# nzfeng/signed-heat-3d

Measured on AMD Instinct MI355X. Metric: grid-nodes/sec end-to-end SHM (conv+PCG), higher is better.
Workload: dtype f64 (Step 1: f64 / packed-f32 tiers)

## Files before the change

### signed-heat-3d_amd/csrc/shm_conv_tiered.hip.h

```cpp
#pragma once
#include "shm_far_carry.h"
#include "shm_kernels.hip.h"

namespace shm {

typedef unsigned uint2v __attribute__((ext_vector_type(2)));
constexpr double kNearA1 = 3.384507729693224e-04;
__device__ __forceinline__ double yukawa_near(double x, double c1, double c2, double m1, const uint2v* __restrict__ tab) {
    const double y0 = __builtin_amdgcn_rsq(x);
    const double t = x * y0;
    const double e2 = fma(-t, y0, 1.0);
    const double cc = fma(e2, c2, c1);
    const double tm = fma(-t, cc, m1);
    const double kf = tm - m1;
    const unsigned ki = (unsigned)__double_as_longlong(tm);
    const double f = fma(-t, cc, -kf);
    const double q = y0 * cc;
    double p = 5.727446245172041e-08;
    p = fma(p, f, kNearA1);
    p = fma(p, f, 1.0);
    uint2v tv = tab[ki & 2047u];
    tv.y += ki << 9;
    return __builtin_bit_cast(double, tv) * (p * q);
}

template <int B>
__device__ __forceinline__ void yukawa_near_batch(const double* __restrict__ x, double c1, double c2, double m1, const uint2v* __restrict__ tab, double* __restrict__ g) {
    double y0[B], t[B], cc[B], q[B], tm[B], f[B], p[B];
    unsigned ki[B];
    uint2v tv[B];
#pragma unroll
    for (int b = 0; b < B; b++) y0[b] = __builtin_amdgcn_rsq(x[b]);
#pragma unroll
    for (int b = 0; b < B; b++) t[b] = x[b] * y0[b];
#pragma unroll
    for (int b = 0; b < B; b++) cc[b] = fma(fma(-t[b], y0[b], 1.0), c2, c1);
#pragma unroll
    for (int b = 0; b < B; b++) tm[b] = fma(-t[b], cc[b], m1);
#pragma unroll
    for (int b = 0; b < B; b++) {
        ki[b] = (unsigned)__double_as_longlong(tm[b]);
        tv[b] = tab[ki[b] & 2047u];
    }
#pragma unroll
    for (int b = 0; b < B; b++) q[b] = y0[b] * cc[b];
#pragma unroll
    for (int b = 0; b < B; b++) f[b] = fma(-t[b], cc[b], -(tm[b] - m1));
#pragma unroll
    for (int b = 0; b < B; b++) p[b] = fma(fma(5.727446245172041e-08, f[b], kNearA1), f[b], 1.0);
#pragma unroll
    for (int b = 0; b < B; b++) p[b] *= q[b];
#pragma unroll
    for (int b = 0; b < B; b++) {
        tv[b].y += ki[b] << 9;
        g[b] = __builtin_bit_cast(double, tv[b]) * p[b];
    }
}

#ifndef SHM_TIER_ASM_BCAST
#define SHM_TIER_ASM_BCAST 1
#endif
__device__ __forceinline__ void pk_fma_lo(float2v& acc, float2v w, float2v g) {
#if SHM_TIER_ASM_BCAST
    asm("v_pk_fma_f32 %0, %1, %2, %0 op_sel_hi:[0,1,1]" : "+v"(acc) : "v"(w), "v"(g));
#else
    acc = __builtin_elementwise_fma(float2v{w.x, w.x}, g, acc);
#endif
}
__device__ __forceinline__ void pk_fma_hi(float2v& acc, float2v w, float2v g) {
#if SHM_TIER_ASM_BCAST
    asm("v_pk_fma_f32 %0, %1, %2, %0 op_sel:[1,0,0] op_sel_hi:[1,1,1]" : "+v"(acc) : "v"(w), "v"(g));
#else
    acc = __builtin_elementwise_fma(float2v{w.y, w.y}, g, acc);
#endif
}

__device__ __forceinline__ int mask_rank(unsigned long long m) {
    return (int)__builtin_amdgcn_mbcnt_hi((unsigned)(m >> 32), __builtin_amdgcn_mbcnt_lo((unsigned)m, 0u));
}

__device__ __forceinline__ double exp2_tab(double u, const uint2v* __restrict__ tab) {
    const double tm = u + 6755399441055744.0;
    const unsigned ki = (unsigned)__double_as_longlong(tm);
    const double f = u - (tm - 6755399441055744.0);
    uint2v tv = tab[ki & 2047u];
    tv.y += ki << 9;
    return __builtin_bit_cast(double, tv) * fma(fma(5.727446245172041e-08, f, kNearA1), f, 1.0);
}

__device__ __forceinline__ float uniform_f32(float v) { return __int_as_float(__builtin_amdgcn_readfirstlane(__float_as_int(v))); }

__device__ __forceinline__ int sample_verdict(unsigned long long* ctr) {
    int v = 0;
    for (unsigned spins = 0; spins < (1u << 20); spins++) {
        v = __builtin_amdgcn_readfirstlane((int)__hip_atomic_load(ctr + 3, __ATOMIC_RELAXED, __HIP_MEMORY_SCOPE_AGENT));
        if (v != 0) break;
        __builtin_amdgcn_s_sleep(32);
    }
    if (v == 0) {
        int r = 0;
        if ((threadIdx.x & 63u) == 0u) {
            unsigned long long expected = 0ull;
            const bool won = __hip_atomic_compare_exchange_strong(ctr + 3, &expected, 2ull, __ATOMIC_RELAXED, __ATOMIC_RELAXED, __HIP_MEMORY_SCOPE_AGENT);
            r = won ? 2 : (int)expected;
        }
        v = __builtin_amdgcn_readfirstlane(r);
    }
    return v == 1;
}
__device__ __forceinline__ void sample_report(unsigned long long* ctr, unsigned long long far_pairs, unsigned long long redo_pairs, int sample_blocks) {
    __hip_atomic_fetch_add(ctr + 0, far_pairs, __ATOMIC_RELAXED, __HIP_MEMORY_SCOPE_AGENT);
    __hip_atomic_fetch_add(ctr + 1, redo_pairs, __ATOMIC_RELAXED, __HIP_MEMORY_SCOPE_AGENT);
    const unsigned long long before = __hip_atomic_fetch_add(ctr + 2, 1ull, __ATOMIC_RELEASE, __HIP_MEMORY_SCOPE_AGENT);
    if (before + 1ull == (unsigned long long)sample_blocks) {
        __builtin_amdgcn_fence(__ATOMIC_ACQUIRE, "agent");
        const unsigned long long farp = __hip_atomic_load(ctr + 0, __ATOMIC_RELAXED, __HIP_MEMORY_SCOPE_AGENT);
        const unsigned long long redo = __hip_atomic_load(ctr + 1, __ATOMIC_RELAXED, __HIP_MEMORY_SCOPE_AGENT);
        unsigned long long expected = 0ull;
        __hip_atomic_compare_exchange_strong(ctr + 3, &expected, (farp > 0ull && redo * 25ull <= farp) ? 1ull : 2ull, __ATOMIC_RELAXED, __ATOMIC_RELAXED, __HIP_MEMORY_SCOPE_AGENT);
    }
}

#ifndef SHM_TIER_TX
#define SHM_TIER_TX 8
#endif
constexpr int kTierTX = SHM_TIER_TX, kTierTY = 64 / kTierTX;
constexpr double kTierBudget = 1.0e-8, kTierEpsFar = 1.0e-6;
constexpr double kTierU0 = 24.0;
constexpr int kTierFlush = 256;
constexpr int kTierCluster = 64;
constexpr int kTierChunk = 4;
constexpr int kTierFill = kTierCluster * kTierChunk;

#ifndef SHM_TIER_FAR_UNROLL
#define SHM_TIER_FAR_UNROLL 4
#endif
#ifndef SHM_TIER_LDS_FETCH
#define SHM_TIER_LDS_FETCH 1
#endif
#ifndef SHM_TIER_LOOKAHEAD
#define SHM_TIER_LOOKAHEAD 1
#endif
#ifndef SHM_TIER_NEAR_BATCH
#define SHM_TIER_NEAR_BATCH 4
#endif
#ifndef SHM_TIER_WAVES_PER_EU
#define SHM_TIER_WAVES_PER_EU 2
#endif
template <int NPT, typename TY, bool CHECK>
__global__ __launch_bounds__(kBlock) __attribute__((amdgpu_waves_per_eu(SHM_TIER_WAVES_PER_EU, SHM_TIER_WAVES_PER_EU))) void conv_tiered_kernel(
    ConvParams P, const double* __restrict__ src , const float* __restrict__ clusters,
    const double* __restrict__ exp_tab_g , TY* __restrict__ Y0, TY* __restrict__ Y1, TY* __restrict__ Y2,
    unsigned long long* __restrict__ counters, unsigned* __restrict__ next_unit ) {
    static_assert(NPT % 2 == 0, "the far tier handles a lane's nodes in packed pairs");
    constexpr int kWaves = kBlock / kWave;
    constexpr int kFarUnroll = SHM_TIER_FAR_UNROLL;
    static_assert(kFarUnroll == kFarGroup, "the carry's bookkeeping (shm_far_carry.h) counts in groups of the far loop's unroll");
    constexpr int kFarList = kTierCluster + kFarGroup;
    static_assert((kTierCluster + kFarGroup - 1 + kFarGroup - 1) / kFarGroup * kFarGroup <= kFarList, "carry + cluster + padding fit the far lists");
    __shared__ double stage64[kWaves][kTierCluster * 6];
    __shared__ __attribute__((aligned(16))) float farA[kWaves][kFarList * 4];
    __shared__ __attribute__((aligned(16))) float farB[kWaves][kFarList * NPT];
    __shared__ __attribute__((aligned(16))) float farC[kWaves][kFarList * 2];
#if SHM_TIER_LDS_FETCH
    __shared__ double2 raw[kWaves][3][kTierCluster];
#endif
    __shared__ uint2v exp_tab[2048];
    __shared__ float4 star_stash[kWaves];
    const int wave = __builtin_amdgcn_readfirstlane((int)(threadIdx.x >> 6)), lane = (int)(threadIdx.x & 63);
    double* const tile = stage64[wave];
    float* const tA = farA[wave];
    float* const tB = farB[wave];
    float* const tC = farC[wave];
    for (int a = threadIdx.x; a < 2048; a += kBlock) {
        uint2v tv = __builtin_bit_cast(uint2v, exp_tab_g[a]);
        tv.y -= (unsigned)a << 9;
        exp_tab[a] = tv;
    }
    __syncthreads();
    const int n = P.n;
    const size_t plane = (size_t)n * n;
    const float lam_l2 = (float)(P.lambda * 1.4426950408889634);
    const float g_l2 = P.tier_log * 1.4426950408889634f;
    const bool drop_on = P.drop_eps_soft > 0.f;
    const float cellq = (float)(P.cell * (P.lambda * 1.4426950408889634));
    const float lws = uniform_f32((float)log2(P.wscale));
    constexpr double kHalfZ = 0.5 * (NPT - 1);
    constexpr double kHalfX = 0.5 * (kTierTX - 1), kHalfY = 0.5 * (kTierTY - 1);
    const float rt_w = (float)(sqrt(kHalfX * kHalfX + kHalfY * kHalfY + kHalfZ * kHalfZ) * P.cell) * 1.000001f;
    const float hx = uniform_f32((float)(kHalfX * P.cell) * 1.000001f), hy = uniform_f32((float)(kHalfY * P.cell) * 1.000001f),
                hz = uniform_f32((float)(kHalfZ * P.cell) * 1.000001f);
    const double c1 = -P.cexp, c2 = -0.5 * P.cexp;
    unsigned long long cnt_near = 0, cnt_far = 0, cnt_redo = 0;
    int decided = -1;
    const unsigned n_units = (unsigned)P.n_tiles;
    const unsigned per_q = (n_units + 7u) / 8u;
    const unsigned my_q = blockIdx.x & 7u;
    unsigned q_off = 0;
    for (;;) {
        unsigned unit = 0xffffffffu;
        while (q_off < 8u) {
            const unsigned q = (my_q + q_off) & 7u;
            const unsigned lo = q * per_q, hi = min(n_units, lo + per_q);
            unsigned t = 0;
            if (lane == 0) t = atomicAdd(next_unit + q, 1u);
            t = (unsigned)__builtin_amdgcn_readfirstlane((int)t);
            if (lo + t < hi) {
                unit = lo + t;
                break;
            }
            q_off++;
        }
        if (unit == 0xffffffffu) break;
        const int tzq = (int)(unit / (unsigned)(P.tiles_x * P.tiles_y)), trem = (int)unit - tzq * (P.tiles_x * P.tiles_y);
        const int tz = P.layer_order ? P.layer_order[tzq] : tzq;
        bool use_diff = false;
        int rule_sel = -1;
        if constexpr (CHECK) {
            use_diff = P.far_rule != 0;
            if (P.unit_rule) {
                rule_sel = (int)P.unit_rule[tzq];
                if (rule_sel == 2) {
                    if (decided < 0) decided = sample_verdict(P.sample_ctr);
                    use_diff = decided != 0;
                } else {
                    use_diff = rule_sel == 1;
                }
            }
        }
        const unsigned long long far_before = cnt_far, redo_before = cnt_redo;
        const int ty = trem / P.tiles_x, tx = trem - ty * P.tiles_x;
        const int i0 = tx * kTierTX, j0 = ty * kTierTY, kk0 = P.kk_begin + tz * NPT;

        double pz0 = 0., ax[NPT], ay[NPT], az[NPT];
        float qz0 = 0.f;
        float2v fx[NPT / 2], fy[NPT / 2], fz[NPT / 2];
        const int li = i0 + (lane % kTierTX), lj = j0 + (lane / kTierTX);
        const int ci = min(li, n - 1), cj = min(lj, n - 1);
        const double px = ci * P.cell + P.bbox_min[0], py = cj * P.cell + P.bbox_min[1];
        const float qx = (float)(px * (P.lambda * 1.4426950408889634)), qy = (float)(py * (P.lambda * 1.4426950408889634));
#pragma unroll
        for (int e = 0; e < NPT; e++) {
            ax[e] = ay[e] = az[e] = 0.;
            fx[e / 2] = fy[e / 2] = fz[e / 2] = float2v{0.f, 0.f};
        }
        pz0 = (P.k0 + kk0 - 1) * P.cell + P.bbox_min[2];
        {
            const long long b = __double_as_longlong(pz0);
            const unsigned lo = (unsigned)__builtin_amdgcn_readfirstlane((int)(unsigned)b), hi = (unsigned)__builtin_amdgcn_readfirstlane((int)(unsigned)(b >> 32));
            pz0 = __longlong_as_double((long long)(((unsigned long long)hi << 32) | lo));
        }
        qz0 = uniform_f32((float)(pz0 * (P.lambda * 1.4426950408889634)));
        const bool live_xy = li < n && lj < n;
        const float cx = uniform_f32((float)((i0 + kHalfX) * P.cell + P.bbox_min[0])), cy = uniform_f32((float)((j0 + kHalfY) * P.cell + P.bbox_min[1]));
        const float cz = uniform_f32((float)((P.k0 + kk0 - 1 + kHalfZ) * P.cell + P.bbox_min[2]));
        float dmin = 3.0e38f, wnear = 0.f, nx = 0.f, ny = 0.f, nz = 0.f;
        for (int s = lane; s < P.S; s += kWave) {
            const double* q = src + (size_t)s * 6;
            const float dx = cx - (float)q[0], dy = cy - (float)q[1], dz = cz - (float)q[2];
            const float w0 = (float)(q[3] * P.wscale), w1 = (float)(q[4] * P.wscale), w2c = (float)(q[5] * P.wscale);
            const float d2 = dx * dx + dy * dy + dz * dz, w2 = w0 * w0 + w1 * w1 + w2c * w2c;
            if (d2 < dmin || (d2 == dmin && w2 > wnear)) {
                dmin = d2;
                wnear = w2;
                nx = dx;
                ny = dy;
                nz = dz;
            }
        }
        {
            auto wave_min_u = [&](unsigned v) {
                v = min(v, (unsigned)__builtin_amdgcn_ds_swizzle((int)v, 0x1f | (1 << 10)));
                v = min(v, (unsigned)__builtin_amdgcn_ds_swizzle((int)v, 0x1f | (2 << 10)));
                v = min(v, (unsigned)__builtin_amdgcn_ds_swizzle((int)v, 0x1f | (4 << 10)));
                v = min(v, (unsigned)__builtin_amdgcn_ds_swizzle((int)v, 0x1f | (8 << 10)));
                v = min(v, (unsigned)__builtin_amdgcn_ds_swizzle((int)v, 0x1f | (16 << 10)));
                return min((unsigned)__builtin_amdgcn_readlane((int)v, 0), (unsigned)__builtin_amdgcn_readlane((int)v, 32));
            };
            const unsigned dbits = wave_min_u(__float_as_uint(dmin));
            const unsigned wkey = __float_as_uint(dmin) == dbits ? ~__float_as_uint(wnear) : 0xffffffffu;
            const unsigned wbits = wave_min_u(wkey);
            const unsigned long long hit = __ballot(wkey == wbits);
            const int win = (int)__builtin_ctzll(hit);
            dmin = __uint_as_float(dbits);
            wnear = __uint_as_float(~wbits);
            nx = __int_as_float(__builtin_amdgcn_readlane(__float_as_int(nx), win));
            ny = __int_as_float(__builtin_amdgcn_readlane(__float_as_int(ny), win));
            nz = __int_as_float(__builtin_amdgcn_readlane(__float_as_int(nz), win));
        }
        dmin = sqrtf(dmin);
        const float fxn = fabsf(nx) + hx, fyn = fabsf(ny) + hy, fzn = fabsf(nz) + hz;
        const float r_hi_w = uniform_f32(sqrtf(fxn * fxn + fyn * fyn + fzn * fzn) * 1.000001f);
        const float lnear_w = uniform_f32(0.5f * __log2f(fmaxf(wnear, 1e-37f)) - 1e-5f);
        const float d0_w = uniform_f32(fmaxf(0.f, dmin * 0.999999f - rt_w));
        const float coff = uniform_f32(lam_l2 * d0_w);

        const int k0 = __builtin_amdgcn_readfirstlane((int)floor((double)d0_w * P.cexp * (1.0 / 2048.0)));
        const double m1 = 6755399441055744.0 - 2048.0 * (double)k0;
        auto far_scale = [&]() {
            float d = d0_w;
            asm volatile("" : "+v"(d));
            return exp2_tab(fma((double)d, P.cexp, -2048.0 * (double)k0), exp_tab) * (P.lambda * 1.4426950408889634) / P.wscale;
        };
        float2v fl[NPT / 2];
#pragma unroll
        for (int e = 0; e < NPT / 2; e++) fl[e] = float2v{0.f, 0.f};
        const float range_c = uniform_f32(2.f * rt_w * lam_l2 - 113.f - coff);
        float star_ux = 0.f, star_uy = 0.f, star_uz = 0.f, star_dc = 0.f, star_inv_d = 0.f;
        if constexpr (CHECK) {
            use_diff = use_diff && coff + 2.f * rt_w * lam_l2 <= 72.f;
        }
        if (use_diff || drop_on) {
            const float inv = dmin > 0.f ? 1.f / dmin : 0.f;
            star_ux = uniform_f32(nx * inv);
            star_uy = uniform_f32(ny * inv);
            star_uz = uniform_f32(nz * inv);
            star_dc = uniform_f32(dmin * 1.000001f);
            const float bx = fmaxf(fabsf(nx) - hx, 0.f), by = fmaxf(fabsf(ny) - hy, 0.f), bz = fmaxf(fabsf(nz) - hz, 0.f);
            const float db = sqrtf(bx * bx + by * by + bz * bz);
            star_inv_d = uniform_f32(dmin > 0.f && db > 0.f ? 1.f / db : __builtin_huge_valf());
        }
        float R_soft = 0.f, R_hard = 0.f;
        if constexpr (CHECK) {
            if (drop_on && lane == 0) star_stash[wave] = float4{(cx - nx) * lam_l2, (cy - ny) * lam_l2, (cz - nz) * lam_l2, wnear};
        }
        const float span_c = uniform_f32(2.f * rt_w * lam_l2 - coff - 960.f);
        int far_pending = 0;
        int carry = 0;
#pragma unroll 1
        for (int pass = 0; pass < 2; pass++) {
#if SHM_TIER_LDS_FETCH
        auto fetch_cluster = [&](int c) {
            const char* g = reinterpret_cast<const char*>(src) + (size_t)c * (kTierCluster * 48);
            const unsigned lo = (unsigned)lane * 48u;
            __builtin_amdgcn_global_load_lds(g + lo, &raw[wave][0][0], 16, 0, 0);
            __builtin_amdgcn_global_load_lds(g + 16 + lo, &raw[wave][1][0], 16, 0, 0);
            __builtin_amdgcn_global_load_lds(g + 32 + lo, &raw[wave][2][0], 16, 0, 0);
        };
#else
        double nq[6];
        auto fetch_cluster = [&](int c) {
            const double* qn = src + ((size_t)c * kTierCluster + lane) * 6;
#pragma unroll
            for (int a = 0; a < 6; a++) nq[a] = qn[a];
        };
#endif
        int cur_batch = -1;
        unsigned long long kept_mask = 0ull, cdrop_mask = 0ull;
        auto load_batch = [&](int b) {
            cur_batch = b;
            const int ci = b * kWave + lane;
            const bool in = ci < P.n_clusters;
            const unsigned long long validm = __ballot(in);
            cdrop_mask = 0ull;
            if (drop_on) {
                const float2* rec = reinterpret_cast<const float2*>(clusters + (size_t)min(ci, P.n_clusters - 1) * kConvClusterRec);
                const float2 r0 = rec[0], r1 = rec[1], r2 = rec[2];
                const float gdx = cx - r0.x, gdy = cy - r0.y, gdz = cz - r1.x;
                const float gap = sqrtf(gdx * gdx + gdy * gdy + gdz * gdz) * 0.999999f - rt_w - r1.y - r_hi_w;
                const float lrel = lws - lnear_w - gap * lam_l2;
                const float lbmax = fmaf(r2.x, 1.4426950408889634f, lrel) + 2e-5f;
                const bool cand = in && gap > 0.f && lbmax <= P.drop_ltau;
                const unsigned long long candm = __ballot(cand);
                if (candm != 0ull) {
                    float bc = cand ? __builtin_amdgcn_exp2f(fmaf(r2.y, 1.4426950408889634f, lrel)) * (r_hi_w * __builtin_amdgcn_rcpf(r_hi_w + gap)) * 1.0001f : 0.f;
                    bc += __int_as_float(__builtin_amdgcn_ds_swizzle(__float_as_int(bc), 0x1f | (1 << 10)));
                    bc += __int_as_float(__builtin_amdgcn_ds_swizzle(__float_as_int(bc), 0x1f | (2 << 10)));
                    bc += __int_as_float(__builtin_amdgcn_ds_swizzle(__float_as_int(bc), 0x1f | (4 << 10)));
                    bc += __int_as_float(__builtin_amdgcn_ds_swizzle(__float_as_int(bc), 0x1f | (8 << 10)));
                    bc += __int_as_float(__builtin_amdgcn_ds_swizzle(__float_as_int(bc), 0x1f | (16 << 10)));
                    const float sum = __int_as_float(__builtin_amdgcn_readlane(__float_as_int(bc), 0)) + __int_as_float(__builtin_amdgcn_readlane(__float_as_int(bc), 32));
                    const float r_new = uniform_f32(R_soft + sum);
                    if (__builtin_amdgcn_readfirstlane((int)(r_new <= P.drop_eps_soft))) {
                        R_soft = r_new;
                        cdrop_mask = candm;
                    } else {
                        cdrop_mask = __ballot(cand && lbmax <= P.drop_ltau_hard);
                        R_hard = uniform_f32(R_hard + (float)(__builtin_popcountll(cdrop_mask) * kTierCluster) * P.drop_tau_hard);
                    }
                }
            }
            kept_mask = pass == 1 ? validm : validm & ~cdrop_mask;
        };
        auto next_kept = [&](int from, bool& cdrop) {
            cdrop = false;
#pragma unroll 1
            while (from < P.n_clusters) {
                const int b = from >> 6;
                if (b != cur_batch) load_batch(b);
                const unsigned long long m = kept_mask & (~0ull << (from & 63));
                if (m != 0ull) {
                    const int bit = (int)__builtin_ctzll(m);
                    cdrop = ((cdrop_mask >> bit) & 1ull) != 0ull;
                    return (b << 6) + bit;
                }
                from = (b + 1) << 6;
            }
            return P.n_clusters;
        };
        R_soft = 0.f;
        R_hard = 0.f;
        bool cdrop_cur = false, cdrop_next = false;
        int c = next_kept(0, cdrop_cur);
        if (c < P.n_clusters) fetch_cluster(c);
#pragma unroll 1
        while (c < P.n_clusters) {
            const int c_next = next_kept(c + 1, cdrop_next);
            const int c_fetch = c_next;
            double q[6];
#if SHM_TIER_LDS_FETCH
            {
                __builtin_amdgcn_s_waitcnt(0x0f70);
                const double2 r0 = raw[wave][0][lane], r1 = raw[wave][1][lane], r2 = raw[wave][2][lane];
                q[0] = r0.x; q[1] = r0.y; q[2] = r1.x; q[3] = r1.y; q[4] = r2.x; q[5] = r2.y;
                __builtin_amdgcn_s_waitcnt(0xc07f);
            }
#else
#pragma unroll
            for (int a = 0; a < 6; a++) q[a] = nq[a];
#endif
            if (c_fetch < P.n_clusters) fetch_cluster(c_fetch);
            unsigned long long nearmask, farmask;
            {
                float q32[6];
#pragma unroll
                for (int a = 0; a < 6; a++) q32[a] = a < 3 ? (float)q[a] : (float)(q[a] * P.wscale);
                const float dx = fmaxf(fabsf(cx - q32[0]) - hx, 0.f), dy = fmaxf(fabsf(cy - q32[1]) - hy, 0.f), dz = fmaxf(fabsf(cz - q32[2]) - hz, 0.f);
                const float dist = sqrtf(dx * dx + dy * dy + dz * dz);
                const float w2 = q32[3] * q32[3] + q32[4] * q32[4] + q32[5] * q32[5];
                const float lw = 0.5f * __log2f(w2);
                const float rel = lw + 1e-5f - lnear_w;
// ... 235 lines not shown
```

### signed-heat-3d_amd/csrc/shm_kernels.hip.h

```cpp
#pragma once
#include <hip/hip_runtime.h>
#include <stdint.h>

#include <type_traits>

#include "shm_constraints.h"
#include "shm_mc_table.h"

namespace shm {

constexpr int kBlock = 256;
constexpr int kMaxPartials = 8192;

__device__ __forceinline__ double wave_sum(double v) {
#pragma unroll
    for (int off = 32; off > 0; off >>= 1) v += __shfl_down(v, off, kWave);
    return v;
}

__device__ __forceinline__ double block_sum(double v, double* lds ) {
    v = wave_sum(v);
    const int lane = threadIdx.x & 63, w = threadIdx.x >> 6;
    if (lane == 0) lds[w] = v;
    __syncthreads();
    double s = 0.;
    if (threadIdx.x == 0) {
        const int nw = (blockDim.x * blockDim.y + 63) >> 6;
        for (int a = 0; a < nw; a++) s += lds[a];
    }
    return s;
}

__device__ __forceinline__ unsigned xcd_remap(unsigned bid, unsigned nblk) {
    const unsigned xcd = bid & 7u, slot = bid >> 3;
    const unsigned q = nblk >> 3, r = nblk & 7u;
    const unsigned base = (xcd < r) ? xcd * (q + 1) : r * (q + 1) + (xcd - r) * q;
    return base + slot;
}

constexpr int kSrcTile = 256;

template <typename T> struct YukawaMath;
template <> struct YukawaMath<double> {
    static constexpr int kExpTabBits = 11;
    static __device__ __forceinline__ double yukawa(double x, double c, const double* __restrict__ tab ) {
        const double y0 = __builtin_amdgcn_rsq(x);
        const double t = x * y0;
        const double e = fma(-t, y0, 1.0);
        const double q = fma(e, 0.375, 0.5) * e;
        const double r = fma(t, q, t);
        const double rinv = fma(y0, q, y0);
        const double tm = fma(r, c, 6755399441055744.0);
        const double kf = tm - 6755399441055744.0;
        const int ki = (int)(unsigned)__double_as_longlong(tm);
        const double f = fma(r, c, -kf);
        double p = 6.461528672932366e-12;
        p = fma(p, f, 5.727446245172041e-08);
        p = fma(p, f, 3.384507717577858e-04);
        p = fma(p, f, 1.0);
        return __builtin_amdgcn_ldexp(tab[ki & ((1 << kExpTabBits) - 1)] * p * rinv, ki >> kExpTabBits);
    }
    static __device__ __forceinline__ double exp_neg(double x) {
        const double kf = rint(x * 1.4426950408889634074);
        double f = fma(kf, -6.93147180369123816490e-01, x);
        f = fma(kf, -1.90821492927058770002e-10, f);
        double p = 1.6059043836821613e-10;
        p = fma(p, f, 2.08767569878681e-09);
        p = fma(p, f, 2.505210838544172e-08);
        p = fma(p, f, 2.755731922398589e-07);
        p = fma(p, f, 2.7557319223985893e-06);
        p = fma(p, f, 2.48015873015873e-05);
        p = fma(p, f, 1.984126984126984e-04);
        p = fma(p, f, 1.3888888888888889e-03);
        p = fma(p, f, 8.333333333333333e-03);
        p = fma(p, f, 4.1666666666666664e-02);
        p = fma(p, f, 1.6666666666666666e-01);
        p = fma(p, f, 0.5);
        p = fma(p, f, 1.0);
        p = fma(p, f, 1.0);
        return __builtin_amdgcn_ldexp(p, (int)kf);
    }
};
template <> struct YukawaMath<float> {
    static __device__ __forceinline__ void rsqrt_and_sqrt(float x, float& rinv, float& r) {
        const float y0 = __builtin_amdgcn_rsqf(x);
        r = x * y0;
        rinv = y0;
    }
    static __device__ __forceinline__ float exp_neg(float x) { return __expf(x); }
};
template <typename T> __device__ __forceinline__ T t_rcp(T x);
template <> __device__ __forceinline__ double t_rcp<double>(double x) { return __builtin_amdgcn_rcp(x); }
template <> __device__ __forceinline__ float t_rcp<float>(float x) { return __builtin_amdgcn_rcpf(x); }
template <typename T> __device__ __forceinline__ T t_sqrt(T x);
template <> __device__ __forceinline__ double t_sqrt<double>(double x) { return sqrt(x); }
template <> __device__ __forceinline__ float t_sqrt<float>(float x) { return sqrtf(x); }

struct ConvParams {
    int n;
    int kk_begin;
    int kk_end;
    int k0;
    int tiles_x, tiles_y;
    double bbox_min[3];
    double cell;
    double lambda;
    double cexp;
    double cexp_inv;
    int S;
    int n_clusters;
    float far_gap;
    float tier_log;
    float skip_base;
    float inv_lambda;
    int exact_offset;
    int n_tiles;
    double wscale;
    float far_redo_ratio;
    int far_rule;
    const unsigned char* unit_rule;
    unsigned long long* sample_ctr;
    int sample_blocks;
    const int* layer_order;
    float drop_eps_soft, drop_ltau, drop_ltau_hard, drop_tau_hard;
    float tier_u0;
    int tier_flush;
    float drop_check;
};

typedef float float2v __attribute__((ext_vector_type(2)));
constexpr int kConvTile = 8;
template <typename T> constexpr int conv_cluster() { return sizeof(T) == 8 ? 64 : 32; }
template <typename T> constexpr int conv_chunk() { return (sizeof(T) == 8 ? kSrcTile : 4 * kSrcTile) / conv_cluster<T>(); }
constexpr int kConvClusterRec = 6;

#ifndef SHM_CONV32_UNROLL
#define SHM_CONV32_UNROLL 2
#endif
template <int NPT> struct ConvSrcUnroll { static constexpr int value = NPT == 8 ? SHM_CONV32_UNROLL : 2; };
template <typename T, int NPT>
__global__ __launch_bounds__(kBlock) void conv_normalize_kernel(ConvParams P, const T* __restrict__ src ,
                                                                const float* __restrict__ src32, const float* __restrict__ clusters,
                                                                const double* __restrict__ exp_tab_g ,
                                                                T* __restrict__ Y0, T* __restrict__ Y1, T* __restrict__ Y2,
                                                                unsigned long long* __restrict__ counters ,
                                                                unsigned* __restrict__ next_tile ) {
    constexpr int kTileZ = (kBlock / 64) * NPT;
    constexpr bool kMixed = sizeof(T) == 8;
    constexpr int kHalves = (!kMixed && NPT == 8) ? 2 : 1;
    constexpr int kNH = NPT / kHalves;
    constexpr int kHalfPlanes = kTileZ / kHalves;
    constexpr int kConvCluster = conv_cluster<T>();
    constexpr int kChunk = conv_chunk<T>();
    constexpr int kFill = kChunk * kConvCluster;
    __shared__ T tile[kFill * 6];
    __shared__ float tile32[kMixed ? kFill * 6 : 1];
    __shared__ float red[kBlock / kWave], redw[kBlock / kWave];
    constexpr int kTab = kMixed ? (1 << YukawaMath<double>::kExpTabBits) : 1;
    __shared__ double exp_tab[kTab];
    if (kMixed)
        for (int a = threadIdx.x; a < kTab; a += kBlock) exp_tab[a] = exp_tab_g[a];
    const int n = P.n;
    const size_t plane = (size_t)n * n;
    unsigned cnt_half64 = 0, cnt_half32 = 0;
    __shared__ int queue_bt;
    auto next_bt = [&](int cur) {
        if (!next_tile) return cur + (int)gridDim.x;
        __syncthreads();
        if (threadIdx.x == 0) queue_bt = (int)atomicAdd(next_tile, 1u);
        __syncthreads();
        return queue_bt;
    };
    for (int bt = next_tile ? next_bt(0) : (int)blockIdx.x; bt < P.n_tiles; bt = next_bt(bt)) {
    __syncthreads();
    const int tz = bt / (P.tiles_x * P.tiles_y), trem = bt - tz * (P.tiles_x * P.tiles_y);
    const int ty = trem / P.tiles_x, tx = trem - ty * P.tiles_x;
    const int i0 = tx * kConvTile, j0 = ty * kConvTile, kk0 = P.kk_begin + tz * kTileZ;

    T pz[NPT], ax[NPT], ay[NPT], az[NPT];
    float qz[NPT], fx[NPT], fy[NPT], fz[NPT];
    bool live[NPT];
    size_t vidx[NPT];
    const int li = i0 + (threadIdx.x & 7), lj = j0 + ((threadIdx.x >> 3) & 7);
    const int ci = min(li, n - 1), cj = min(lj, n - 1);
    const double xd = ci * P.cell + P.bbox_min[0], yd = cj * P.cell + P.bbox_min[1];
    const T px = (T)xd, py = (T)yd;
    const float qx = (float)xd, qy = (float)yd;
#pragma unroll
    for (int e = 0; e < NPT; e++) {
        int kk = kk0 + (int)(threadIdx.x >> 6) + e * (kBlock / 64);
        live[e] = li < n && lj < n && kk < P.kk_end;
        kk = min(kk, P.kk_end - 1);
        vidx[e] = (size_t)kk * plane + (size_t)cj * n + ci;
        const int k = P.k0 + kk - 1;
        const double z = k * P.cell + P.bbox_min[2];
        pz[e] = (T)z;
        qz[e] = (float)z;
        ax[e] = ay[e] = az[e] = (T)0;
        fx[e] = fy[e] = fz[e] = 0.f;
    }
    constexpr double kHalfZ = 0.5 * (kHalfPlanes - 1);
    const float cx = (float)((i0 + 3.5) * P.cell + P.bbox_min[0]), cy = (float)((j0 + 3.5) * P.cell + P.bbox_min[1]);
    const float rt = (float)(sqrt(3.5 * 3.5 * 2 + kHalfZ * kHalfZ) * P.cell) * 1.000001f;
    float cz[kHalves], ln_anear[kHalves], r_hi[kHalves], d0t[kHalves];
#pragma unroll
    for (int h = 0; h < kHalves; h++) {
        cz[h] = (float)((P.k0 + kk0 + h * kHalfPlanes - 1 + kHalfZ) * P.cell + P.bbox_min[2]);
        float dmin = 3.0e38f, wnear = 0.f;
        for (int s = threadIdx.x; s < P.S; s += kBlock) {
            const float dx = cx - (float)src[(size_t)s * 6], dy = cy - (float)src[(size_t)s * 6 + 1], dz = cz[h] - (float)src[(size_t)s * 6 + 2];
            const float wx = (float)src[(size_t)s * 6 + 3], wy = (float)src[(size_t)s * 6 + 4], wz = (float)src[(size_t)s * 6 + 5];
            const float d2 = dx * dx + dy * dy + dz * dz, w2 = wx * wx + wy * wy + wz * wz;
            if (d2 < dmin || (d2 == dmin && w2 > wnear)) {
                dmin = d2;
                wnear = w2;
            }
        }
#pragma unroll
        for (int off = 32; off > 0; off >>= 1) {
            const float od = __shfl_xor(dmin, off, kWave), ow = __shfl_xor(wnear, off, kWave);
            if (od < dmin || (od == dmin && ow > wnear)) {
                dmin = od;
                wnear = ow;
            }
        }
        if (h > 0) __syncthreads();
        if ((threadIdx.x & 63) == 0) {
            red[threadIdx.x >> 6] = dmin;
            redw[threadIdx.x >> 6] = wnear;
        }
        __syncthreads();
        dmin = red[0];
        wnear = redw[0];
#pragma unroll
        for (int a = 1; a < kBlock / kWave; a++)
            if (red[a] < dmin || (red[a] == dmin && redw[a] > wnear)) {
                dmin = red[a];
                wnear = redw[a];
            }
        dmin = sqrtf(dmin);
        ln_anear[h] = 0.5f * __logf(fmaxf(wnear, 1e-37f)) - 1e-5f;
        r_hi[h] = dmin * 1.000001f + rt;
        d0t[h] = fmaxf(0.f, dmin * 0.999999f - rt);
    }

    T d0[NPT];
#pragma unroll
    for (int e = 0; e < NPT; e++) d0[e] = kMixed ? (T)0 : (T)d0t[e / kNH];
    if (!kMixed && P.exact_offset) {
        float m2[NPT];
#pragma unroll
        for (int e = 0; e < NPT; e++) m2[e] = 3.0e38f;
        for (int s0 = 0; s0 < P.S; s0 += kFill) {
            const int cnt = min(kFill, P.S - s0);
            __syncthreads();
            for (int a = threadIdx.x; a < cnt * 6; a += kBlock) tile[a] = src[(size_t)s0 * 6 + a];
            __syncthreads();
            for (int s = 0; s < cnt; s++) {
                const float dx = qx - (float)tile[6 * s], dy = qy - (float)tile[6 * s + 1];
                const float dxy2 = dx * dx + dy * dy;
#pragma unroll
                for (int e = 0; e < NPT; e++) {
                    const float dz = qz[e] - (float)tile[6 * s + 2];
                    m2[e] = fminf(m2[e], dxy2 + dz * dz);
                }
            }
        }
#pragma unroll
        for (int e = 0; e < NPT; e++) d0[e] = (T)(sqrtf(m2[e]) * 0.99999f);
    }
    const float lamf = (float)P.lambda;
    const float cexp32 = (float)(-P.lambda * 1.4426950408889634);
    float coff[NPT];
#pragma unroll
    for (int e = 0; e < NPT; e++) coff[e] = (float)(P.lambda * 1.4426950408889634 * (double)d0[e]);
    for (int c0 = 0; c0 < P.n_clusters; c0 += kChunk) {
        const int ncl = min(kChunk, P.n_clusters - c0);
        const int cnt = ncl * kConvCluster;
        auto record_gap = [&](const float* rec, int h) {
            const float gdx = cx - rec[0], gdy = cy - rec[1], gdz = cz[h] - rec[2];
// ... 1640 lines not shown
```

### signed-heat-3d_amd/csrc/shm_solver.hip.h

```cpp
#pragma once
#include "shm_host.hip.h"
#include "shm_kernels.hip.h"
#include "shm_conv_tiered.hip.h"
#include "shm_cg_fused.hip.h"
#include "shm_twolevel.hip.h"
#include "shm_schur.hip.h"
#include "shm_dct.hip.h"
#include "shm_dct_gemm.hip.h"
#include "shm_green_fft.hip.h"
#include "shm_sample.hip.h"
#include "shm_audit.hip.h"
#include "shm_iso_indexed.hip.h"
#include "shm_raycast.hip.h"
#include "shm_redistance.hip.h"
#include "shm_plan.h"

namespace shm {

template <typename T> constexpr int vec_width() { return sizeof(T) == 8 ? 2 : 4; }

template <typename T>
struct Slab {
    int k0 = 0, k1 = 0, nzl = 0;
    size_t plane = 0, nown = 0, ntot = 0;
// ... 497 lines not shown
        in.full_wanted = full_wanted(); in.fft_available = fft_available(); in.gemm_dct = gemm_dct(); in.fused_available = fused_available();
        in.step1 = step1_kernel(); in.conv_est_total_ms = conv_est_total_ms;
        if (o) {
            in.solver = o->solver; in.preconditioner = o->preconditioner; in.dual_form = o->dual_form;
            in.step1_budget = o->step1_budget; in.fast = o->fast_integration != 0;
        }
        in.knobs = plan_knobs(knob);
        return in;
    }
    void select_step1_arith(int arith) {
        if (arith != SHM_STEP1_AUTO && arith != SHM_STEP1_EXACT_F64 && arith != SHM_STEP1_REFERENCE_F64) throw Error(SHM_ERR_INVALID, "unknown step1_arith");
        conv_reference = sizeof(T) == 8 && arith == SHM_STEP1_REFERENCE_F64;
        conv_tiered = sizeof(T) == 8 && arith == SHM_STEP1_AUTO && knob("SHM_CONV_EXACT") == nullptr && tier_exponent_span_ok();
        conv_tier_exact = sizeof(T) == 8 && arith == SHM_STEP1_EXACT_F64 && knob("SHM_CONV_EXACT_CLASSIC") == nullptr && tier_exponent_span_ok(true);
        conv_tiered = conv_tiered || conv_tier_exact;
        conv_tiered32 = sizeof(T) == 4 && knob("SHM_CONV32_CLASSIC") == nullptr && tier_exponent_span_ok();
        step1_selected = sizeof(T) == 4 || (conv_tiered && !conv_tier_exact) ? SHM_STEP1_AUTO : conv_reference ? SHM_STEP1_REFERENCE_F64 : SHM_STEP1_EXACT_F64;
    }
    bool tier_exponent_span_ok(bool every_pair = false) const {
        const double rt = std::sqrt(2 * 3.5 * 3.5 + 1.5 * 1.5) * cell;
        const double reach = every_pair ? lambda * std::sqrt(3.0) * (double)(n - 1) * cell : std::min((sizeof(T) == 8 ? conv_tier_skip_base : conv_skip_base) + 2.0794415416798357, 1.0e6);
        const double bits = (4.0 * rt * lambda + reach + std::max(conv_w_span, 43.0)) * 1.4426950408889634 + 16.0;
        return bits < 990.0;
    }
    void need_problem() const {
        if (!have_problem) throw Error(SHM_ERR_STATE, "shm_grid_set_problem has not been called");
    }

    const int* layer_order_for(Slab<T>& sl, int kk_begin, int layers, int npt) {
        const bool off = knob("SHM_TIER_LAYER_ORDER") != nullptr && atoi(knob("SHM_TIER_LAYER_ORDER")) == 0;
        if (off || layers < 16) return nullptr;
        const long long key = ((long long)kk_begin << 40) ^ ((long long)layers << 20) ^ ((long long)npt << 8) ^ (long long)sl.k0 * 0x9E3779B1LL;
        if (sl.layer_order.p && sl.layer_order_key == key) return sl.layer_order.p;
        std::vector<std::pair<double, int>> byc((size_t)layers);
        for (int l = 0; l < layers; l++) byc[(size_t)l] = {std::fabs((double)(sl.k0 + kk_begin - 1 + l * npt) + 0.5 * (npt - 1) - 0.5 * (n - 1)), l};
        std::stable_sort(byc.begin(), byc.end());
        std::vector<int> order;
        order.reserve((size_t)layers);
        for (int q = 0; q < 8; q++)
            for (int r = q; r < layers; r += 8) order.push_back(byc[(size_t)r].second);
        sl.layer_order.upload(order, stream);
        sl.layer_order_key = key;
        return sl.layer_order.p;
    }
    int far_rule_now() const {
        const char* e = knob("SHM_TIER_FAR_RULE");
        if (e) return atoi(e) != 0;
        return 0;
    }
    bool far_rule_plan(Slab<T>& sl, int planes, int npt) {
        if (sizeof(T) != 8 || !conv_tiered || conv_tier_exact || slabs.size() != 1 || total_slabs != 1 || knob("SHM_TIER_FAR_RULE") != nullptr) return false;
        if (step1_budget > 0. && step1_budget != kTierBudget) return false;
        const int layers = (planes + npt - 1) / npt;
        if (layers < 64 || layers % 8 != 0 || planes % npt != 0) return false;
        const long long key = ((long long)layers << 32) ^ ((long long)npt << 16);
        if (sl.sample_key != key) {
            std::vector<char> role((size_t)layers, 2);
            std::vector<int> A, B1;
            const int nA = 8;
            for (int a = 0; a < nA; a++) {
                const int l = (int)(((long long)(2 * a + 1) * layers) / (2 * nA));
                A.push_back(l);
                role[(size_t)l] = 1;
            }
            std::vector<std::pair<double, int>> byc;
            for (int l = 0; l < layers; l++)
                if (role[(size_t)l] != 1) byc.push_back({std::fabs((double)(sl.k0 + l * npt) + 0.5 * (npt - 1) - 0.5 * (n - 1)), l});
            std::stable_sort(byc.begin(), byc.end());
            for (int a = 0; a < 8; a++) B1.push_back(byc[(size_t)a].second);
            std::vector<int> order;
            std::vector<unsigned char> rule;
            size_t next_rest = 8;
            std::vector<std::vector<int>> rest(8);
            {
                std::vector<int> want(8);
                for (int q = 0; q < 8; q++) want[(size_t)q] = layers / 8 - 1 - ((nA == 8 || q % 2 == 0) ? 1 : 0);
                bool any = true;
                while (any && next_rest < byc.size()) {
                    any = false;
                    for (int q = 0; q < 8 && next_rest < byc.size(); q++)
                        if ((int)rest[(size_t)q].size() < want[(size_t)q]) {
                            rest[(size_t)q].push_back(byc[next_rest++].second);
                            any = true;
                        }
                }
            }
            for (int q = 0, a = 0; q < 8; q++) {
                if (nA == 8 || q % 2 == 0) {
                    order.push_back(A[(size_t)a++]);
                    rule.push_back(1);
                }
                order.push_back(B1[(size_t)q]);
                rule.push_back(0);
                for (int l : rest[(size_t)q]) {
                    order.push_back(l);
                    rule.push_back(2);
                }
            }
            if ((int)order.size() != layers) throw Error(SHM_ERR_INVALID, "far_rule_plan: internal count mismatch");
            sl.sample_blocks = nA * ((n + kTierTX - 1) / kTierTX) * ((n + kTierTY - 1) / kTierTY);
            sl.sample_order.upload(order, stream);
            sl.sample_rule.upload(rule, stream);
            sl.sample_ctr.alloc(4);
            sl.sample_key = key;
        }
        return true;
    }
    void launch_conv() {
        const bool slab_log = knob("SHM_CONV_SLAB_LOG") != nullptr;
        Event slab_ev[2];
        unsigned long long slab_pairs_seen[2] = {0, 0};
        for (Slab<T>& sl : slabs) {
            if (slab_log) {
                HIPCHK(hipStreamSynchronize(stream));
                slab_ev[0].record(stream);
            }
            ConvParams P;
            P.layer_order = nullptr;
            P.unit_rule = nullptr;
            P.sample_ctr = nullptr;
            P.sample_blocks = 0;
            P.far_rule = conv_tiered && !conv_tier_exact && sizeof(T) == 8 ? far_rule_now() : 0;
            P.n = n;
            P.kk_begin = 1;
            P.kk_end = sl.nzl + 1;
            P.k0 = sl.k0;
            for (int a = 0; a < 3; a++) P.bbox_min[a] = bbox_min[a] - conv_ctr[a];
            P.cell = cell;
            P.lambda = lambda;
            P.cexp = -lambda * 2954.639443740597;
            P.cexp_inv = 1.0 / std::fabs(P.cexp);
            P.S = n_clusters * conv_cluster<T>();
            P.n_clusters = n_clusters;
            P.far_gap = conv_reference ? 3.0e38f : (float)conv_far_gap;
            const double budget = step1_budget > 0. ? step1_budget : kTierBudget;
            const double g_shift = std::log(budget / kTierBudget);
            P.tier_log = conv_tier_exact ? 3.0e38f : conv_tiered32 ? -1.0e30f : (float)std::max(2.0, conv_tier_log - g_shift);
            P.wscale = conv_wscale;
            {
                const double ratio = budget / kTierEpsFar;
                P.far_redo_ratio = ratio > 0. ? (float)ratio : 3.0e38f;
            }
            P.skip_base = conv_tier_exact || conv_reference ? 3.0e38f : (float)std::min(conv_tiered ? conv_tier_skip_base - g_shift : conv_skip_base, 3.0e38);
            {
                const double eps = conv_tier_exact ? 0. : sizeof(T) == 8 ? conv_drop_eps64 * (budget / kTierBudget) : conv_drop_eps32;
                const double eps_soft = 0.875 * eps, tau = eps_soft / conv_drop_K, tau_hard = 0.125 * eps / (double)std::max<int64_t>(1, S);
                P.drop_eps_soft = (float)eps_soft;
                P.drop_ltau = eps > 0. ? (float)std::log2(tau) : -3.0e38f;
                P.drop_ltau_hard = eps > 0. ? (float)std::log2(tau_hard) : -3.0e38f;
                P.drop_tau_hard = (float)(tau_hard * 1.0001);
                P.drop_check = P.far_redo_ratio < 1.0e30f ? (float)((double)P.far_redo_ratio / budget) : (float)(1.0 / kTierEpsFar);
                P.tier_u0 = (float)kTierU0;
                P.tier_flush = kTierFlush;
            }
            P.inv_lambda = (float)(1.0 / lambda);
            P.tiles_x = (n + kConvTile - 1) / kConvTile;
            P.tiles_y = P.tiles_x;
            const int planes = P.kk_end - P.kk_begin;
            const bool npt4 = (long long)P.tiles_x * P.tiles_y * ((planes + 15) / 16) >= conv_grid_cap;
            const bool npt4_env = knob("SHM_CONV_NPT4") != nullptr;
            const bool npt8 = sizeof(T) == 4 && !npt4_env && npt4 && (long long)P.tiles_x * P.tiles_y * ((planes + 31) / 32) >= conv_grid_cap;
            const int tile_z = npt8 ? 32 : npt4 ? 16 : 8;
            const double half_z = 0.5 * ((npt8 ? 16 : tile_z) - 1);
            const double tile_diam = 2.0 * std::sqrt(2 * 3.5 * 3.5 + half_z * half_z) * cell;
            P.exact_offset = (lambda * tile_diam > 30.0) ? 1 : 0;
            const int tiles_z = (planes + tile_z - 1) / tile_z;
            P.n_tiles = P.tiles_x * P.tiles_y * tiles_z;
            unsigned grid = (unsigned)std::min(P.n_tiles, conv_grid_cap);
            {
                int occ = 0;
                const void* kfn = npt4 ? reinterpret_cast<const void*>(conv_normalize_kernel<T, 4>) : reinterpret_cast<const void*>(conv_normalize_kernel<T, 2>);
                if constexpr (sizeof(T) == 4)
                    if (npt8) kfn = reinterpret_cast<const void*>(conv_normalize_kernel<float, 8>);
                if (conv_tiered) kfn = npt4 ? reinterpret_cast<const void*>(conv_tiered_kernel<4, double, true>) : reinterpret_cast<const void*>(conv_tiered_kernel<2, double, true>);
                if (conv_tiered32) kfn = npt4 ? reinterpret_cast<const void*>(conv_tiered_kernel<4, float, false>) : reinterpret_cast<const void*>(conv_tiered_kernel<2, float, false>);
                if (hipOccupancyMaxActiveBlocksPerMultiprocessor(&occ, kfn, kBlock, 0) != hipSuccess || occ < 1) occ = 2;
                const unsigned resident = (unsigned)(occ * num_cus);
                const double pairs = (double)sl.nown * (double)S;
                const double conv_est_ms = pairs / (sizeof(T) == 8 ? 1.2e9 : 3.5e9);
                conv_est_total_ms = (&sl == &slabs[0] ? 0. : conv_est_total_ms) + conv_est_ms;
                const double setup_est_ms = 2.2e-3 * (double)std::min<int64_t>(S, (int64_t)8 * n * n);
                if (conv_tiered || conv_tiered32) grid = std::min(grid, resident);
                if (!o_fast_hint && conv_est_ms < 4.0 * setup_est_ms && grid > resident - resident / 8) grid = resident - resident / 8;
            }
            const bool uniform_tiles = lambda * cell * n < 100.;
            const int want_chunks = (conv_tiered || conv_tiered32) ? 1 : (uniform_tiles && conv_est_total_ms >= 10. ? std::min(16, (int)std::lround(conv_est_total_ms / 2.5)) : 1);
            const int nchunks = std::max(1, std::min(tiles_z, want_chunks));
            const int chunk_planes = ((tiles_z + nchunks - 1) / nchunks) * tile_z;
            if (!d_pair_counters.p) d_pair_counters.alloc(3);
            if (!d_unit_counters.p) d_unit_counters.alloc(8 * kMaxConvLaunches);
            if (&sl == &slabs[0]) {
                HIPCHK(hipMemsetAsync(d_pair_counters.p, 0, 3 * sizeof(unsigned long long), stream));
                HIPCHK(hipMemsetAsync(d_unit_counters.p, 0, 8 * kMaxConvLaunches * sizeof(unsigned), stream));
                conv_launch_index = 0;
                conv_launches_last = 0;
            }
            unsigned long long* const cnt = d_pair_counters.p;
            auto launch_range = [&](int b0, int b1, int sel, int rule = -1, const int* order = nullptr, int order_layers = 0) {
                if (b1 <= b0) return;
                conv_launches_last++;
                const int tz_sel = 4 * sel;
                ConvParams Pc = P;
                Pc.kk_begin = 1 + b0;
                Pc.kk_end = std::min(sl.nzl + 1, 1 + b1);
                Pc.n_tiles = P.tiles_x * P.tiles_y * ((Pc.kk_end - Pc.kk_begin + tz_sel - 1) / tz_sel);
                const dim3 g((unsigned)std::min<long long>(Pc.n_tiles, grid));
                if (conv_tiered || conv_tiered32) {
                    if (conv_launch_index >= kMaxConvLaunches) throw Error(SHM_ERR_INVALID, "too many Step-1 launches");
                    unsigned* const head = d_unit_counters.p + 8 * conv_launch_index++;
                    const int npt = npt4 ? 4 : 2;
                    Pc.tiles_x = (n + kTierTX - 1) / kTierTX;
                    Pc.tiles_y = (n + kTierTY - 1) / kTierTY;
                    const int layers = order ? order_layers : (Pc.kk_end - Pc.kk_begin + npt - 1) / npt;
                    Pc.n_tiles = Pc.tiles_x * Pc.tiles_y * layers;
                    Pc.layer_order = order ? order : layer_order_for(sl, Pc.kk_begin, layers, npt);
                    if (rule >= 0) Pc.far_rule = rule;
                    const dim3 gt((unsigned)std::min<long long>((Pc.n_tiles + 3) / 4, grid));
                    if constexpr (sizeof(T) == 8) {
                        if (npt4)
                            hipLaunchKernelGGL((conv_tiered_kernel<4, double, true>), gt, dim3(kBlock), 0, stream, Pc, d_src.p, d_clusters.p, d_exptab.p, sl.Y0.p, sl.Y1.p, sl.Y2.p, cnt, head);
                        else
                            hipLaunchKernelGGL((conv_tiered_kernel<2, double, true>), gt, dim3(kBlock), 0, stream, Pc, d_src.p, d_clusters.p, d_exptab.p, sl.Y0.p, sl.Y1.p, sl.Y2.p, cnt, head);
                    } else {
                        Pc.S = n_clusters_t * kTierCluster;
                        Pc.n_clusters = n_clusters_t;
                        if (npt4)
                            hipLaunchKernelGGL((conv_tiered_kernel<4, float, false>), gt, dim3(kBlock), 0, stream, Pc, d_src_t.p, d_clusters_t.p, d_exptab.p, sl.Y0.p, sl.Y1.p, sl.Y2.p, cnt, head);
                        else
                            hipLaunchKernelGGL((conv_tiered_kernel<2, float, false>), gt, dim3(kBlock), 0, stream, Pc, d_src_t.p, d_clusters_t.p, d_exptab.p, sl.Y0.p, sl.Y1.p, sl.Y2.p, cnt, head);
                    }
                    return;
                }
                unsigned* head = nullptr;
                if (conv_launch_index < kMaxConvLaunches) head = d_unit_counters.p + 8 * conv_launch_index++;
                if constexpr (sizeof(T) == 4) {
                    if (sel == 8) {
                        hipLaunchKernelGGL((conv_normalize_kernel<float, 8>), g, dim3(kBlock), 0, stream, Pc, d_src.p, d_src32.p, d_clusters.p, d_exptab.p, sl.Y0.p, sl.Y1.p,
                                           sl.Y2.p, cnt, head);
                        return;
                    }
                }
                if (sel >= 4)
                    hipLaunchKernelGGL((conv_normalize_kernel<T, 4>), g, dim3(kBlock), 0, stream, Pc, d_src.p, d_src32.p, d_clusters.p, d_exptab.p, sl.Y0.p, sl.Y1.p, sl.Y2.p, cnt, head);
                else
                    hipLaunchKernelGGL((conv_normalize_kernel<T, 2>), g, dim3(kBlock), 0, stream, Pc, d_src.p, d_src32.p, d_clusters.p, d_exptab.p, sl.Y0.p, sl.Y1.p, sl.Y2.p, cnt, head);
            };
            const int sel0 = npt8 ? 8 : npt4 ? 4 : 2;
            if (sizeof(T) == 4 && !conv_tiered32 && nchunks == 1 && sel0 > 2 && planes % tile_z != 0) {
                int b = (planes / tile_z) * tile_z;
                launch_range(0, b, sel0);
                for (int sel = sel0 / 2; sel >= 2; sel /= 2) {
                    const int tz_sel = 4 * sel, take = sel > 2 ? ((planes - b) / tz_sel) * tz_sel : planes - b;
                    launch_range(b, b + take, sel);
                    b += take;
                }
            } else if (far_rule_plan(sl, planes, npt4 ? 4 : 2)) {
                const int npt = npt4 ? 4 : 2, layers = planes / npt;
                HIPCHK(hipMemsetAsync(sl.sample_ctr.p, 0, 4 * sizeof(unsigned long long), stream));
                P.unit_rule = sl.sample_rule.p;
                P.sample_ctr = sl.sample_ctr.p;
                P.sample_blocks = sl.sample_blocks;
                launch_range(0, planes, sel0, 0, sl.sample_order.p, layers);
                P.unit_rule = nullptr;
            } else {
                for (int b0 = 0; b0 < planes; b0 += chunk_planes) launch_range(b0, std::min(planes, b0 + chunk_planes), sel0);
            }
            if (slab_log) {
                slab_ev[1].record(stream);
                HIPCHK(hipStreamSynchronize(stream));
                unsigned long long h[2] = {0, 0};
                HIPCHK(hipMemcpy(h, d_pair_counters.p, sizeof h, hipMemcpyDeviceToHost));
                fprintf(stderr, "[shm] step1 slab planes [%d,%d) ms %.3f pairs_fp64 %.6e pairs_fp32 %.6e\n", sl.k0, sl.k1, elapsed(slab_ev[0], slab_ev[1]),
                        (double)(h[0] - slab_pairs_seen[0]), (double)(h[1] - slab_pairs_seen[1]));
                slab_pairs_seen[0] = h[0];
                slab_pairs_seen[1] = h[1];
            }
        }
        HIPCHK(hipGetLastError());
        exchange_Y_halos();
        have_conv = true;
        last_step1_arith = step1_selected;
        last_step1_budget = sizeof(T) == 8 && conv_tiered && !conv_tier_exact ? (step1_budget > 0. ? step1_budget : kTierBudget) : 0.;
    }
    void exchange_Y_halos() {
        if (total_slabs <= 1) return;
        for (int sel : {ARR_Y0, ARR_Y1, ARR_Y2}) halo_exchange(sel);
    }

    void launch_div(int scrub) {
        for (Slab<T>& sl : slabs) {
            if (vec == 1) {
                hipLaunchKernelGGL((divergence_kernel<T>), dim3((unsigned)((n + kBlock - 1) / kBlock), (unsigned)n, (unsigned)sl.nzl), dim3(kBlock), 0, stream, sl.gp,
                                   sl.Y0.p, sl.Y1.p, sl.Y2.p, sl.r.p, scrub);
                sl.div_sum_blocks = 0;
                continue;
            }
            constexpr int V = vec_width<T>();
            const DivGeometry g = div_geometry(sl);
            sl.div_partials.alloc(g.nblk);
            sl.div_sum_blocks = (int)g.nblk;
            hipLaunchKernelGGL((divergence_march_kernel<T, V>), dim3(g.nblk), dim3(kBlock), 0, stream, sl.gp, g.LX, g.xchunks, g.rowgroups, g.ZC, sl.Y0.p, sl.Y1.p, sl.Y2.p,
                               sl.r.p, scrub, sl.div_partials.p);
        }
        HIPCHK(hipGetLastError());
        have_div = true;
    }
// ... 2419 lines not shown
```

Measured before the change: 697.2 million.

## Prune nearest-source scan with cluster bounding-sphere bounds in tiered conv

```diff
diff --git a/signed-heat-3d_amd/csrc/shm_cluster_verdict.h b/signed-heat-3d_amd/csrc/shm_cluster_verdict.h
--- /dev/null
+++ b/signed-heat-3d_amd/csrc/shm_cluster_verdict.h
@@ -0,0 +1,31 @@
+#pragma once
+#include <math.h>
+
+#ifdef __HIPCC__
+#define SHM_CLUSTER_HD __host__ __device__ __forceinline__
+#else
+#define SHM_CLUSTER_HD inline
+#endif
+
+namespace shm {
+
+struct ScanBounds {
+    float lo;
+    float hi;
+};
+
+SHM_CLUSTER_HD ScanBounds scan_prune_bounds(float cx, float cy, float cz, float mx, float my, float mz, float rad) {
+    const float dx = cx - mx, dy = cy - my, dz = cz - mz;
+    const float d = sqrtf(dx * dx + dy * dy + dz * dz);
+    const float slack = 1.0e-6f * (fabsf(cx) + fabsf(cy) + fabsf(cz) + fabsf(mx) + fabsf(my) + fabsf(mz) + rad);
+    ScanBounds b;
+    b.lo = d * 0.999999f - rad - slack;
+    b.hi = d * 1.000001f + rad + slack;
+    return b;
+}
+
+SHM_CLUSTER_HD float scan_first_look_bound(float d2min) { return sqrtf(d2min) * 1.000001f; }
+
+SHM_CLUSTER_HD bool scan_keeps(float lo, float U) { return !(lo > U); }
+
+}
diff --git a/signed-heat-3d_amd/csrc/shm_conv_tiered.hip.h b/signed-heat-3d_amd/csrc/shm_conv_tiered.hip.h
--- a/signed-heat-3d_amd/csrc/shm_conv_tiered.hip.h
+++ b/signed-heat-3d_amd/csrc/shm_conv_tiered.hip.h
@@ -1,4 +1,5 @@
 #pragma once
+#include "shm_cluster_verdict.h"
 #include "shm_far_carry.h"
 #include "shm_kernels.hip.h"
 
@@ -255,8 +256,16 @@
         const float cx = uniform_f32((float)((i0 + kHalfX) * P.cell + P.bbox_min[0])), cy = uniform_f32((float)((j0 + kHalfY) * P.cell + P.bbox_min[1]));
         const float cz = uniform_f32((float)((P.k0 + kk0 - 1 + kHalfZ) * P.cell + P.bbox_min[2]));
         float dmin = 3.0e38f, wnear = 0.f, nx = 0.f, ny = 0.f, nz = 0.f;
-        for (int s = lane; s < P.S; s += kWave) {
-            const double* q = src + (size_t)s * 6;
+        auto wave_min_u = [&](unsigned v) {
+            v = min(v, (unsigned)__builtin_amdgcn_ds_swizzle((int)v, 0x1f | (1 << 10)));
+            v = min(v, (unsigned)__builtin_amdgcn_ds_swizzle((int)v, 0x1f | (2 << 10)));
+            v = min(v, (unsigned)__builtin_amdgcn_ds_swizzle((int)v, 0x1f | (4 << 10)));
+            v = min(v, (unsigned)__builtin_amdgcn_ds_swizzle((int)v, 0x1f | (8 << 10)));
+            v = min(v, (unsigned)__builtin_amdgcn_ds_swizzle((int)v, 0x1f | (16 << 10)));
+            return min((unsigned)__builtin_amdgcn_readlane((int)v, 0), (unsigned)__builtin_amdgcn_readlane((int)v, 32));
+        };
+        auto scan_cluster = [&](int k) {
+            const double* q = src + ((size_t)k * kWave + lane) * 6;
             const float dx = cx - (float)q[0], dy = cy - (float)q[1], dz = cz - (float)q[2];
             const float w0 = (float)(q[3] * P.wscale), w1 = (float)(q[4] * P.wscale), w2c = (float)(q[5] * P.wscale);
             const float d2 = dx * dx + dy * dy + dz * dz, w2 = w0 * w0 + w1 * w1 + w2c * w2c;
@@ -267,16 +276,52 @@
                 ny = dy;
                 nz = dz;
             }
+        };
+        if (P.block_shortcuts) {
+            auto batch_bounds = [&](int b, bool& in) {
+                const int ci = b * kWave + lane;
+                in = ci < P.n_clusters;
+                const float2* rec = reinterpret_cast<const float2*>(clusters + (size_t)min(ci, P.n_clusters - 1) * kConvClusterRec);
+                const float2 r0 = rec[0], r1 = rec[1];
+                return scan_prune_bounds(cx, cy, cz, r0.x, r0.y, r1.x, r1.y);
+            };
+            const int n_batches = (P.n_clusters + kWave - 1) / kWave;
+            float ub = __builtin_huge_valf();
+            int ub_k = 0;
+#pragma unroll 1
+            for (int b = 0; b < n_batches; b++) {
+                bool in;
+                const ScanBounds sb = batch_bounds(b, in);
+                if (in && sb.hi < ub) {
+                    ub = sb.hi;
+                    ub_k = b * kWave + lane;
+                }
+            }
+            const unsigned ubits = wave_min_u(__float_as_uint(ub));
+            const int k_first = __builtin_amdgcn_readlane(ub_k, (int)__builtin_ctzll(__ballot(__float_as_uint(ub) == ubits)));
+            float U = __uint_as_float(ubits);
+            {
+                const double* q = src + ((size_t)k_first * kWave + lane) * 6;
+                const float dx = cx - (float)q[0], dy = cy - (float)q[1], dz = cz - (float)q[2];
+                const float d2 = dx * dx + dy * dy + dz * dz;
+                U = fminf(U, scan_first_look_bound(__uint_as_float(wave_min_u(__float_as_uint(d2)))));
+            }
+#pragma unroll 1
+            for (int b = 0; b < n_batches; b++) {
+                bool in;
+                const ScanBounds sb = batch_bounds(b, in);
+                unsigned long long m = __ballot(in && scan_keeps(sb.lo, U));
+#pragma unroll 1
+                while (m != 0ull) {
+                    scan_cluster(b * kWave + (int)__builtin_ctzll(m));
+                    m &= m - 1ull;
+                }
+            }
+        } else {
+#pragma unroll 1
+            for (int k = 0; k < P.n_clusters; k++) scan_cluster(k);
         }
         {
-            auto wave_min_u = [&](unsigned v) {
-                v = min(v, (unsigned)__builtin_amdgcn_ds_swizzle((int)v, 0x1f | (1 << 10)));
-                v = min(v, (unsigned)__builtin_amdgcn_ds_swizzle((int)v, 0x1f | (2 << 10)));
-                v = min(v, (unsigned)__builtin_amdgcn_ds_swizzle((int)v, 0x1f | (4 << 10)));
-                v = min(v, (unsigned)__builtin_amdgcn_ds_swizzle((int)v, 0x1f | (8 << 10)));
-                v = min(v, (unsigned)__builtin_amdgcn_ds_swizzle((int)v, 0x1f | (16 << 10)));
-                return min((unsigned)__builtin_amdgcn_readlane((int)v, 0), (unsigned)__builtin_amdgcn_readlane((int)v, 32));
-            };
             const unsigned dbits = wave_min_u(__float_as_uint(dmin));
             const unsigned wkey = __float_as_uint(dmin) == dbits ? ~__float_as_uint(wnear) : 0xffffffffu;
             const unsigned wbits = wave_min_u(wkey);
diff --git a/signed-heat-3d_amd/csrc/shm_kernels.hip.h b/signed-heat-3d_amd/csrc/shm_kernels.hip.h
--- a/signed-heat-3d_amd/csrc/shm_kernels.hip.h
+++ b/signed-heat-3d_amd/csrc/shm_kernels.hip.h
@@ -126,6 +126,7 @@
     float tier_u0;
     int tier_flush;
     float drop_check;
+    int block_shortcuts;
 };
 
 typedef float float2v __attribute__((ext_vector_type(2)));
diff --git a/signed-heat-3d_amd/csrc/shm_solver.hip.h b/signed-heat-3d_amd/csrc/shm_solver.hip.h
--- a/signed-heat-3d_amd/csrc/shm_solver.hip.h
+++ b/signed-heat-3d_amd/csrc/shm_solver.hip.h
@@ -673,6 +673,10 @@
                 P.drop_check = P.far_redo_ratio < 1.0e30f ? (float)((double)P.far_redo_ratio / budget) : (float)(1.0 / kTierEpsFar);
                 P.tier_u0 = (float)kTierU0;
                 P.tier_flush = kTierFlush;
+            }
+            {
+                const char* bs = knob("SHM_TIER_BLOCK_SHORTCUTS");
+                P.block_shortcuts = bs == nullptr || atoi(bs) != 0;
             }
             P.inv_lambda = (float)(1.0 / lambda);
             P.tiles_x = (n + kConvTile - 1) / kConvTile;
```

After: 696.1 million. No clear change (-0.2%).
